# dotchen/LAV

Hardware: AMD Instinct MI355X
Metric: frames/s full agent fwd (32k-pt LiDAR + 3 cams) (higher is better)
Workload: dtype f32 (convolution contractions on the matrix cores with f32 accumulate at the error of an fp32 dot product, DESIGN 4.3: the layers on the split-operand kernel - BEV backbone, heads, crop stems, the brake net's mid-size layers - and ERFNet's persistent runs of pairs as two power-of-two-scaled fp16 pie

## Files before the change

include/lav_amd.h:

```cpp
#ifndef LAV_AMD_H
#define LAV_AMD_H

#include <stddef.h>
#include <stdint.h>

#ifdef __cplusplus
extern "C" {
#endif

#define LAV_ABI_VERSION 43

#define LAV_OK 0
#define LAV_EINVAL (-1)
#define LAV_EHIP (-2)
#define LAV_EWORKSPACE (-3)

int lav_abi_version(void);
const char *lav_last_error(void);
int lav_device_count(void);

int lav_profile_enable(int slots);
int lav_profile_reset(void);
int lav_profile_read(const char *kernel, double *total_ms, int *launches);

typedef struct lav_grid {
    float min_x, max_x, min_y, max_y;
    float ppm;
    int nx, ny;
} lav_grid;

typedef struct lav_pointnet {
    const float *w1, *b1, *w2, *b2;
    int num_input;
    int channels;
} lav_pointnet;

size_t lav_pillar_workspace_bytes(int batch, int max_points, const lav_grid *grid);
int lav_pillar_workspace_init(void *workspace, size_t workspace_bytes, void *stream);

int lav_pillar_scatter(const float *points, const int *h_num_points, int batch, int max_points, int D,
                       const lav_grid *grid, const lav_pointnet *net, float *canvas,
                       int *unique_coords, int *inverse, int *counts,
                       void *workspace, size_t workspace_bytes, void *stream);
// ... 75 lines not shown
                float *shift, void *stream);
int lav_conv_tile_info(const lav_conv *c, int *info);
size_t lav_conv_workspace_bytes(const lav_conv *c);
int lav_conv2d(const lav_conv *c, const float *x, const float *w_packed, const float *bias, const float *scale,
               const float *shift, const float *residual, float *y, void *workspace, size_t workspace_bytes,
               void *stream);
#define LAV_AMAX_PARTS 512
int lav_absmax_parts(const float *x, long n, float *parts, void *stream);
int lav_conv_amax_count(const lav_conv *c);
int lav_conv2d_amax(const lav_conv *c, const float *x, const float *w_packed, const float *bias, const float *scale,
                    const float *shift, const float *residual, float *y, void *workspace, size_t workspace_bytes,
                    const float *amax_in, int amax_in_count, float *amax_out, void *stream);

int lav_deconv_grouped(int batch, int cin, int h, int w, int groups, const int *cout_per_group, int kernel, int stride,
                       int pad, int out_pad, const float *x, const float *weight, const float *bias, int sigmoid_from,
                       float *y, void *stream);

int lav_crop_rotate(const float *feat, int feat_batch, int C, int H, int W, const float *locs, const float *oris, int n,
                    float pixels_per_meter, int crop, float offset_x, float offset_y, float *out, void *stream);
int lav_crop_rotate_indexed(const float *feat, int num_maps, const int *map_index, int C, int H, int W, const float *locs,
                            const float *oris, int n, float pixels_per_meter, int crop, float offset_x, float offset_y,
                            float *out, void *stream);
int lav_crop_rotate_backward(const float *grad_out, int num_maps, const int *map_index, int C, int H, int W, const float *locs,
                             const float *oris, int n, float pixels_per_meter, int crop, float offset_x, float offset_y,
                             float *grad_feat, void *stream);

int lav_merge_ticks(const float *tick, float *prev, int rows, int dim, float *cur, void *stream);
int lav_stack_sweeps(const float *fused, float *ring, const long *d_slot, const long *d_sweeps, const float *d_R,
                     const float *d_t, int num_sweeps, int rows, int dim, float *out, void *stream);
size_t lav_extract_peaks_workspace_bytes(int ncls, int h, int w);
int lav_extract_peaks(const float *heat, int ncls, int h, int w, int ks, int max_det, int apply_sigmoid,
                      const float *size, int size_c, const float *ori, int ori_c, float *out, void *workspace,
                      size_t workspace_bytes, void *stream);

int lav_attn_pool(const float *x, int batch, int C, int N, int heads, const float *u, const float *dots_bias,
                  const float *w_v, const float *b_v, float *out, void *stream);

size_t lav_attn_train_workspace_bytes(int batch, int C, int N, int heads);
int lav_attn_train_forward(const float *x, int batch, int C, int N, int heads, const float *q, const float *w_kv, const float *b_kv,
                           const float *pe, float scale, float *u, float *dots_bias, float *out, float *p, float *xbar, void *stream);
int lav_attn_train_backward(const float *x, int batch, int C, int N, int heads, const float *q, const float *w_kv, const float *b_kv,
                            const float *pe, float scale, const float *u, const float *p, const float *xbar, const float *dout, float *dx,
                            float *dq, float *dw_kv, float *db_kv, void *workspace, size_t workspace_bytes, void *stream);

int lav_nonfinite_count(int n, const float *const *tensors, const long *numel, int *counter2, void *stream);

int lav_maxpool3x3s2(const float *x, int batch, int channels, int h, int w, float *y, void *stream);
int lav_channel_affine(const float *x, int batch, int channels, long plane, const float *scale, const float *shift, float *y, void *stream);
int lav_copy_many(int n, const void *const *src, void *const *dst, const size_t *bytes, void *stream);
int lav_stage_many(int n, const void *const *src, float *const *dst, const int *dims, const long *strides, const int *src_is_u8,
                   void *stream);
int lav_stage_many_block(int n, const void *const *src, float *const *dst, const int *dims, const long *strides, const int *src_is_u8,
                         const void *block, int block_bytes, void *block_dst, void *stream);

int lav_linear_act(const float *x, int batch, int in_features, const float *weight, const float *bias, int out_features,
                   int act, float *out, void *stream);

int lav_det_decode(const float *rows, int ncls, int max_det, int cls, double min_score, double ego_x, double ego_y,
                   double near_px, double far_px, double min_box, double cx, double cy, double skip_px, double ppm,
                   float *actors, int *n_out, void *stream);
int lav_batch_limit(const int *d_rows);
int lav_det_decode_report(const float *rows, int ncls, int max_det, int cls, double min_score, double ego_x, double ego_y,
                          double near_px, double far_px, double min_box, double cx, double cy, double skip_px, double ppm,
                          float *actors, int *n_out, float *host_rows, int *host_n, unsigned *host_seq, void *stream);

size_t lav_pillar_decorate_workspace_bytes(int batch, int max_points, const lav_grid *grid);
// ... 182 lines not shown
```

lav_amd/_lib.py:

```python
from __future__ import annotations

import ctypes as C
import os

HERE = os.path.dirname(os.path.abspath(__file__))
LIB_PATH = os.environ.get("LAV_AMD_LIB") or os.path.join(HERE, "liblav_amd.so")

ABI_VERSION = 43
MAX_CAM = 4
MAX_CAM_F64 = 8


class Grid(C.Structure):
    _fields_ = [("min_x", C.c_float), ("max_x", C.c_float), ("min_y", C.c_float), ("max_y", C.c_float),
                ("ppm", C.c_float), ("nx", C.c_int), ("ny", C.c_int)]


class PointNet(C.Structure):
    _fields_ = [("w1", C.c_void_p), ("b1", C.c_void_p), ("w2", C.c_void_p), ("b2", C.c_void_p),
                ("num_input", C.c_int), ("channels", C.c_int)]


class Camera(C.Structure):
    _fields_ = [("K", C.c_float * 9), ("l2w", C.c_float * 16), ("w2c", C.c_float * 16)]


class CameraF64(C.Structure):
    _fields_ = [("l2w", C.c_double * 16), ("w2c", C.c_double * 16), ("K", C.c_double * 9)]


class Conv(C.Structure):
    _fields_ = [(n, C.c_int) for n in (
        "batch", "in_c_total", "in_c_offset", "cin", "h", "w", "cout", "kh", "kw", "stride", "pad_h", "pad_w",
        "dil_h", "dil_w", "transposed", "out_pad", "out_c_total", "out_c_offset", "relu_pre", "relu_post", "sigmoid", "target_cus")] + [("pad_value", C.c_float), ("precision", C.c_int)]


CONV_F32, CONV_BF16X6, CONV_F16X3 = 1, 2, 3


_P, _I, _Z, _F = C.c_void_p, C.c_int, C.c_size_t, C.c_float
SIGNATURES = {
# ... 77 lines not shown
    "lav_bn_train_forward_mask": (_I, [_P, _P, _P, _P, _I, _I, C.c_long, _P, _P, C.c_double, _I, _P, _P, _P, _P, _P, _Z, _P]),
    "lav_bn_train_backward_mask": (_I, [_P, _P, _P, _P, _I, _I, C.c_long, _P, _P, _P, _I, _P, _P, _P, _P, _P, _P, _Z, _P]),
    "lav_pair_train_supported": (_I, [_I, _I]),
    "lav_pair_train_workspace_bytes": (_Z, [_I, _I, _I]),
    "lav_pair_train_forward": (_I, [_P, _P, _P, _P, _P, _I, _I, _I, _I, _I, _P, _P, _P]),
    "lav_pair_train_backward": (_I, [_P, _P, _P, _P, _P, _I, _I, _I, _I, _I, _P, _P, _P, _P, _P, _P, _P, _Z, _P]),
    "lav_seg_xent_workspace_bytes": (_Z, []),
    "lav_seg_xent_forward": (_I, [_P, _P, _I, _I, C.c_long, _P, _P, _P, _Z, _P]),
    "lav_seg_xent_up_forward": (_I, [_P, _P, _I, _I, _I, _I, _I, _I, _P, _P, _P, _Z, _P]),
    "lav_attn_train_workspace_bytes": (_Z, [_I, _I, _I, _I]),
    "lav_attn_train_forward": (_I, [_P, _I, _I, _I, _I, _P, _P, _P, _P, C.c_float, _P, _P, _P, _P, _P, _P]),
    "lav_attn_train_backward": (_I, [_P, _I, _I, _I, _I, _P, _P, _P, _P, C.c_float, _P, _P, _P, _P, _P, _P, _P, _P, _P, _Z, _P]),
    "lav_bn_train_forward": (_I, [_P, _P, _P, _I, _I, C.c_long, _P, _P, C.c_double, _I, _I, _P, _P, _P, _P, _Z, _P]),
    "lav_bn_train_backward": (_I, [_P, _P, _P, _I, _I, C.c_long, _P, _P, _P, _I, _I, _P, _P, _P, _P, _P, _Z, _P]),
    "lav_bn_train_amax_count": (_I, [_I, _I, C.c_long]),
    "lav_bn_train_forward_amax": (_I, [_P, _P, _P, _I, _I, C.c_long, _P, _P, C.c_double, _I, _I, _P, _P, _P, _P, _P, _Z, _P]),
    "lav_bn_train_backward_amax": (_I, [_P, _P, _P, _I, _I, C.c_long, _P, _P, _P, _I, _I, _P, _P, _P, _P, _P, _P, _Z, _P]),
    "lav_attn_pool": (_I, [_P, _I, _I, _I, _I, _P, _P, _P, _P, _P, _P]),
    "lav_linear_act": (_I, [_P, _I, _I, _P, _P, _I, _I, _P, _P]),
    "lav_maxpool3x3s2": (_I, [_P, _I, _I, _I, _I, _P, _P]),
    "lav_channel_affine": (_I, [_P, _I, _I, C.c_long, _P, _P, _P, _P]),
    "lav_nonfinite_count": (_I, [_I, C.POINTER(_P), C.POINTER(C.c_long), _P, _P]),
    "lav_copy_many": (_I, [_I, C.POINTER(_P), C.POINTER(_P), C.POINTER(_Z), _P]),
    "lav_stage_many": (_I, [_I, C.POINTER(_P), C.POINTER(_P), C.POINTER(_I), C.POINTER(C.c_long), C.POINTER(_I), _P]),
    "lav_det_decode": (_I, [_P, _I, _I, _I] + [C.c_double] * 10 + [_P, _P, _P]),
    "lav_det_decode_report": (_I, [_P, _I, _I, _I] + [C.c_double] * 10 + [_P, _P, _P, _P, _P, _P]),
    "lav_stage_many_block": (_I, [_I, C.POINTER(_P), C.POINTER(_P), C.POINTER(_I), C.POINTER(C.c_long), C.POINTER(_I), _P, _I, _P, _P]),
    "lav_batch_limit": (_I, [_P]),
    "lav_pool_affine": (_I, [_P, _I, _I, _I, _I, _P, _P, _I, _P, _I, _I, _P]),
    "lav_merge_ticks": (_I, [_P, _P, _I, _I, _P, _P]),
    "lav_stack_sweeps": (_I, [_P, _P, _P, _P, _P, _P, _I, _I, _I, _P, _P]),
    "lav_extract_peaks_workspace_bytes": (_Z, [_I, _I, _I]),
    "lav_extract_peaks": (_I, [_P, _I, _I, _I, _I, _I, _I, _P, _I, _P, _I, _P, _P, _Z, _P]),
    "lav_augment_u8": (_I, [_P, _P, _I, _I, _I, _P, C.c_ulonglong, _P]),
    "lav_bev_stack_u8": (_I, [_P, _P, _P, _P, _I, _I, _I, _I, _P]),
    "lav_bev_stack_tile_paths": (_I, [C.POINTER(C.c_double), C.POINTER(_I), _I, _I, C.POINTER(_I)]),
    "lav_debug_view": (_I, [_P, _I, _I, _P, _I, _I, _P, _I, _I, _P, _I, _P, _I, _P, _I, _P, _P, _P, C.c_double, C.c_double, _I, C.c_double, C.c_double, _I,
                            _I, _I, _P, _P, _P]),
    "lav_log_view": (_I, [_P, _I, _P, _I, _P, _P, _I, _I, _P, _P, _I, _P, _I, _I, _P, _P]),
    "lav_eval_acc_words": (_Z, [_I]),
    "lav_eval_frame": (_I, [_P, _P, _P, _I, _I, _F, _P, _I, _P, _P, _I, _I, _I, _P, _P, _I, _P, _P, _P, _I] + [C.c_double] * 6 + [_I, _P, _P]),
    "lav_eval_seg": (_I, [_P, _P, _I, _I, _I, _I, _I, _P, _P]),
    "lav_eval_scores": (_I, [_P, _P, _I, C.c_double, _I, _P, _P]),
    "lav_eval_plans_words": (_Z, [_I]),
    "lav_eval_plans": (_I, [_P, _P, _P, _P, _P, _P, _I, _I, _I, _P, _P, _P, _I, _P, _P]),
    "lav_eval_distill_words": (_Z, [_I]),
    "lav_eval_distill": (_I, [_P] * 8 + [_I, _I, _I] + [_P] * 5 + [_I, _P, _P]),
    "lav_eval_drive_words": (_Z, [_I]),
    "lav_eval_drive": (_I, [_P, _P, _P, _I, _I, _I, _I, _P, _P, _I, _P, _P, _I, _I] + [C.c_double] * 6 + [_I, _P, _P]),
    "lav_jpeg_scan_capacity": (C.c_longlong, [_I, _I, _I]),
    "lav_jpeg_workspace_bytes": (_Z, [_I, _I, _I, _I]),
    "lav_jpeg_encode": (_I, [_P, _I, _I, _I, _I, _P, _I, _P, C.c_longlong, _P, _P, _Z, _P]),
}

_lib = None


def load() -> C.CDLL:
    global _lib
    if _lib is not None:
        return _lib
    if not os.path.exists(LIB_PATH):
        raise RuntimeError(
            f"{LIB_PATH} not found: build it with `python -m lav_amd.build` (hipcc, gfx950). "
            "lav_amd has no CPU or pure-torch fallback.")
    lib = C.CDLL(LIB_PATH)
# ... 24 lines not shown
```

lav_amd/build.py:

```python
from __future__ import annotations

import os
import subprocess
import sys
import time

HERE = os.path.dirname(os.path.abspath(__file__))
REPO = os.path.dirname(HERE)
CSRC = os.path.join(HERE, "csrc")
LIB = os.path.join(HERE, "liblav_amd.so")
SOURCES = ["misc.hip", "pillar.hip", "paint.hip", "paint_frames.hip", "gru.hip", "gru_seq.hip", "conv.hip", "conv_f16.hip", "conv_pair.hip", "conv_run.hip", "conv_tile.hip", "deconv.hip", "crop.hip", "frame.hip", "attn.hip", "bn_train.hip", "conv_wgrad.hip", "upconv.hip", "conv_pair_train.hip", "augment.hip", "bev_stack.hip", "debug_view.hip", "log_view.hip", "eval_metrics.hip", "eval_camera.hip", "eval_plans.hip", "eval_drive.hip", "eval_distill.hip", "jpeg.hip"]
EXTRA_FLAGS = {"pillar.hip": ["-ffp-contract=off"], "paint.hip": ["-ffp-contract=off"], "paint_frames.hip": ["-ffp-contract=off"], "crop.hip": ["-ffp-contract=off"],
               "frame.hip": ["-ffp-contract=off"], "augment.hip": ["-ffp-contract=off"], "bev_stack.hip": ["-ffp-contract=off"],
               "debug_view.hip": ["-ffp-contract=off", "-fhip-fp32-correctly-rounded-divide-sqrt"],
               "log_view.hip": ["-ffp-contract=off"],
               "eval_metrics.hip": ["-ffp-contract=off"],
               "eval_plans.hip": ["-ffp-contract=off"],
               "eval_drive.hip": ["-ffp-contract=off"],
               "eval_distill.hip": ["-ffp-contract=off"]}
FLAGS = ["--offload-arch=gfx950", "-O3", "-std=c++17", "-fPIC", "-Wall", "-Wno-unused-function", "-fno-slp-vectorize",
         "-I", os.path.join(REPO, "include"), "-I", CSRC]


def _hipcc() -> str:
    for c in (os.environ.get("HIPCC"), "/opt/rocm/bin/hipcc", "hipcc"):
        if c and (os.path.isabs(c) and os.path.exists(c) or not os.path.isabs(c)):
            return c
    raise RuntimeError("hipcc not found")


def needs_build() -> bool:
    if not os.path.exists(LIB):
        return True
    t = os.path.getmtime(LIB)
    deps = [os.path.join(CSRC, f) for f in os.listdir(CSRC)] + [os.path.join(REPO, "include", "lav_amd.h")]
    return any(os.path.getmtime(d) > t for d in deps)


def build(force: bool = False, verbose: bool = True) -> str:
    if not force and not needs_build():
        return LIB
    objs = []
    procs = []
    os.makedirs(os.path.join(HERE, "build"), exist_ok=True)
# ... 24 lines not shown
```

lav_amd/frame.py:

```python
from __future__ import annotations

import math
import os
import time
from collections import deque

import numpy as np
import torch

from . import ops
from .model_inference import InferModel

GAP = 5
_COPY_STREAM = os.environ.get("LAV_COPY_STREAM", "0") == "1"
_DET_REPORT = os.environ.get("LAV_DET_REPORT", "1") != "0"
_POSE_BLOCK = os.environ.get("LAV_POSE_BLOCK", "1") != "0"
_BRAKE_AFTER = os.environ.get("LAV_BRAKE_AFTER", "in")
_BRAKE_SPLIT = os.environ.get("LAV_BRAKE_SPLIT", "wide")
if _BRAKE_SPLIT in ("0", "off", "none"):
    _BRAKE_SPLIT = ""
_DIAG_SKIP = set(filter(None, os.environ.get("LAV_DIAG_SKIP", "").split(",")))


def ego_box_mask(lidar: torch.Tensor) -> torch.Tensor:
    x, y, z = lidar[:, 0], lidar[:, 1], lidar[:, 2]
    return (x > -2.4) & (x < 0) & (y > -0.8) & (y < 0.8) & (z > -1.5) & (z < -1)


def move_lidar_points(xyz: torch.Tensor, dloc, ori0: float, ori1: float) -> torch.Tensor:
    dloc = np.asarray(dloc, np.float64) @ np.array([[math.cos(ori0), -math.sin(ori0)], [math.sin(ori0), math.cos(ori0)]])
    ori = ori1 - ori0
    c, s_ = float(np.float32(math.cos(ori))), float(np.float32(math.sin(ori)))
    x, y = xyz[:, 0], xyz[:, 1]
    return torch.stack([(x * c + y * -s_) + float(np.float32(dloc[0])), (x * s_ + y * c) + float(np.float32(dloc[1])),
                        xyz[:, 2]], dim=1)


def _at_frame_precision(fn):
    import functools

    @functools.wraps(fn)
    def wrapped(self, *a, **k):
        with ops.precision(self.precision):
            return fn(self, *a, **k)
    return wrapped


class FramePipeline:
    def __init__(self, lidar_model, uniplanner, seg_model, bra_model, camera_x=1.5, camera_z=2.4, num_frame_stack=2,
                 device=torch.device("cuda"), compact_ego_box: bool = False):
        self.device = device
        self.precision = ops.frame_precision()
        self.infer_model = InferModel(lidar_model, uniplanner, camera_x, camera_z, device=device, precision=self.precision)
        self.seg_model, self.bra_model = seg_model, bra_model
        self.num_frame_stack = num_frame_stack
        self.num_frame_keep = (num_frame_stack + 1) * GAP
        self.compact_ego_box = compact_ego_box
        self.reset()

    def reset(self):
        self.lidars, self.locs, self.oris = deque(), deque(), deque()
        self.prev_lidar = None

    def _sem_probs(self, all_rgbs):
        probs = getattr(self.seg_model, "probs", None)
        return probs(all_rgbs) if probs is not None else torch.softmax(self.seg_model(all_rgbs), dim=1)

    def preprocess(self, lidar):
        m = ego_box_mask(lidar)
        if self.compact_ego_box:
            return lidar[~m]
        out = lidar.clone()
        out[:, 0] = torch.where(m, torch.full_like(out[:, 0], float("nan")), out[:, 0])
        return out

    def get_stacked_lidar(self):
        loc0, ori0 = self.locs[-1], self.oris[-1]
        parts = []
        for i, t in enumerate(range(len(self.lidars) - 1, -1, -GAP)):
            lidar = self.lidars[t]
            xyz = move_lidar_points(lidar[:, :3], self.locs[t] - loc0, ori0, self.oris[t])
            onehot = torch.zeros((len(xyz), self.num_frame_stack + 1), dtype=xyz.dtype, device=xyz.device)
            onehot[:, i] = 1
            parts.append(torch.cat([xyz, lidar[:, 3:], onehot], dim=-1))
        return torch.cat(parts)

# ... 80 lines not shown

    def _grow(self, new_p: int):
        torch.cuda.synchronize()
        f = dict(dtype=torch.float32, device=self.device)
        old_p = self.P
        b_tick = torch.full((new_p, 4), float("nan"), **f)
        b_prev = torch.full((new_p, 4), float("nan"), **f); b_prev[:old_p] = self.b_prev
        ring = torch.full((self.num_frame_keep, 2 * new_p, 8), float("nan"), **f); ring[:, :2 * old_p] = self.ring
        self.b_tick, self.b_prev, self.ring, self.P = b_tick, b_prev, ring, new_p
        self.graphs.clear(); self.outs.clear()
        torch.cuda.synchronize()

    def reset(self):
        super().reset()
        if hasattr(self, "ring"):
            self.ring.fill_(float("nan")); self.b_prev.fill_(float("nan"))
            self.frame_no = 0
            self.poses = deque()

    def _g_lidar(self):
        im, lm = self.infer_model, self.infer_model.lidar_model
        cur = ops.merge_ticks(self.b_tick, self.b_prev)
        pred_sem = self._sem_probs(self.b_all_rgbs)
        fused = im.forward_paint(cur, pred_sem)
        lidar_points = ops.stack_sweeps(fused, self.ring, self.b_slot, self.b_sweeps, self.b_R, self.b_t)
        canvas = lm.point_pillar_net([lidar_points], [lidar_points.shape[0]])
        if self.b_features is None:
            self.b_features = torch.empty((1, lm.backbone.out_channels, canvas.shape[2] // 2, canvas.shape[3] // 2),
                                          dtype=torch.float32, device=canvas.device)
        lm.backbone(canvas, out=self.b_features)
        return dict(lidar_points=lidar_points)

    def _g_heads(self):
        heat, size, ori, pred_bev = self.infer_model.lidar_model.heads(self.b_features)
        det_raw = ops.extract_peaks(heat[0], size[0], ori[0], apply_sigmoid=True)
        if self.device_others:
            im, up = self.infer_model, self.infer_model.uniplanner
            ox, oy = up.offsets()
            H, W = im._bev_hw
            ops.det_decode(det_raw, self.d_actors, self.d_n, cls=1, min_score=0.2, ego_xy=(160, 280), near_px=2.0,
                           far_px=30 * im.pixels_per_meter, min_box=0.1 * im.pixels_per_meter,
                           centre_xy=(float(W / 2 + ox * W / 2), float(H / 2 + oy * H / 2)), skip_px=4.0, ppm=up.pixels_per_meter,
                           report=(self.h_det, self.h_n, self.h_seq) if _DET_REPORT else None)
            if self.forced_others is not None:
                self.d_actors.copy_(self.forced_others[0]); self.d_n.copy_(self.forced_others[1])
        return dict(det_raw=det_raw, pred_bev=pred_bev)

    def set_forced_others(self, locs=None, oris=None):
        if not self.device_others:
            raise RuntimeError("set_forced_others needs the device-resident others branch")
        if locs is None:
            self.forced_others = None
        else:
            n = len(locs)
            host = torch.zeros((45,), dtype=torch.float32)
            host[:2 * n] = torch.as_tensor(locs, dtype=torch.float32).reshape(-1)
            host[30:30 + n] = torch.as_tensor(oris, dtype=torch.float32).reshape(-1)
            self.forced_others = (host.to(self.device), torch.tensor([n], dtype=torch.int32, device=self.device), n)
        torch.cuda.synchronize()
        self.graphs.pop("heads", None); self.outs.pop("heads", None)

    def _g_brake(self):
        pred_bra = self.bra_model(self.b_rgbs, self.b_tel)
        ops.nonfinite_count([pred_bra], self.d_health)
        return dict(pred_bra=pred_bra)

    def _g_brake_a(self):
        first = self.b_rgbs if _BRAKE_SPLIT == "wide" else self.b_tel
# ... 303 lines not shown
```

lav_amd/lidar.py:

```python
from __future__ import annotations

import torch
from torch import nn
import torch.nn.functional as F

from . import _lib
from . import ops
from .engine import Engine, _bn_tuple
from .ops import Amax, ConvLayer, ConvRun, ConvTileRun, GroupedDeconv, PointwiseUpconv
from .point_pillar import PointPillarNet

_NORM = dict(eps=1e-3, momentum=0.01)


def _stage(cin, cout, n):
    mods = []
    for j in range(n):
        mods += [nn.Conv2d(cin if j == 0 else cout, cout, 3, 2 if j == 0 else 1, 1, bias=False),
                 nn.ReLU(inplace=True), nn.BatchNorm2d(cout, **_NORM)]
    return nn.Sequential(*mods)


def _up(cin, cout, k, s, p=0, op=0):
    return nn.Sequential(nn.ConvTranspose2d(cin, cout, k, s, p, op, bias=False), nn.ReLU(inplace=True),
# ... 148 lines not shown
        self.seg_head = Head(6 * nf, 3, output_activation=torch.sigmoid)

    def _head_engine(self, names, device):
        prec = ops.infer_precision()
        if prec == 0 and getattr(self, "heads_precision", 0):
            prec = self.heads_precision
        def build():
            hs = [getattr(self, n) for n in names]
            for h in hs:
                if not (h._sigmoid or isinstance(h.output_activation, nn.Identity)):
                    raise RuntimeError("Head.output_activation must be identity or sigmoid for the fused epilogue")
            sig = [h._sigmoid for h in hs]
            if any(sig[:-1]):
                raise RuntimeError("fused head deconvolution expects the sigmoid head last")
            w = lambda: torch.cat([h.net[0].weight.detach() for h in hs], dim=0)
            bn = lambda: tuple(torch.cat([getattr(h.net[2], n).detach() for h in hs]) for n in ("running_mean", "running_var", "weight", "bias"))
            cts = [h.net[3] for h in hs]
            outs = [ct.weight.shape[1] for ct in cts]
            return dict(outs=outs,
                        conv=ConvLayer(w, padding=1, bn=bn, bn_eps=hs[0].net[2].eps, relu_pre=True, device=device,
                                       precision=prec),
                        deconv=GroupedDeconv(cts, sigmoid_from=sum(outs[:-1]) if sig[-1] else -1, device=device))
        return self._engine_for(device, (names, prec), build)

    ALL_HEADS = ("center_head", "box_head", "ori_head", "seg_head")

    def heads(self, features, names=ALL_HEADS):
        if self.training:
            return self._heads_train(features, names)
        e = self._head_engine(tuple(names), features.device)
        fused = e["deconv"](e["conv"](features, amax_in=ops.amax_of(features)))
        return tuple(torch.split(fused, e["outs"], dim=1))

    def _heads_train(self, features, names):
        hs = [getattr(self, n) for n in names]
        if len(hs) == 1 or not features.is_cuda:
            return tuple(h(features) for h in hs)
        from .train.hipnn import bn_act_many, conv2d
        mid = conv2d(features, torch.cat([h.net[0].weight for h in hs], dim=0), 1, 1)
        mid = bn_act_many([h.net[2] for h in hs], mid, relu_pre=True)
        outs, off = [], 0
        for h in hs:
            c = h.net[0].out_channels
            outs.append(h.output_activation(h.net[3](mid[:, off:off + c])))
            off += c
        return tuple(outs)

    def forward(self, lidars, num_points):
        features = self.backbone(self.point_pillar_net(lidars, num_points))
        return (features, *self.heads(features))
```

lav_amd/model_inference.py:

```python
from __future__ import annotations

import numpy as np
import torch
import torch.nn as nn
from torch.nn import functional as F

from . import ops
from .planner_common import crop_feature, transform_points

CAMERA_YAWS = [-60, 0, 60]


def carla_matrix(x, y, z, yaw_deg=0.0):
    f = np.float32
    a = f(yaw_deg) * (f(np.pi) / f(180.0))
    c, s = np.cos(a, dtype=f), np.sin(a, dtype=f)
    return np.array([[c, -s, 0, x], [s, c, 0, y], [0, 0, 1, z], [0, 0, 0, 1]], f)


def carla_inverse_matrix(x, y, z, yaw_deg=0.0):
    f = np.float32
    a = f(yaw_deg) * (f(np.pi) / f(180.0))
    c, s = np.cos(a, dtype=f), np.sin(a, dtype=f)
    ax, ay, az = -f(x), -f(y), -f(z)
# ... 7 lines not shown

    def __init__(self, cam_yaw, lidar_xyz=(0, 0, 2.5), cam_xyz=(1.4, 0, 2.5), rgb_h=320, rgb_w=320, fov=60):
        super().__init__()
        focal = rgb_w / (2.0 * np.tan(fov * np.pi / 360.0))
        K = torch.eye(3)
        K[0, 0] = K[1, 1] = focal
        K[0, 2] = rgb_w / 2.0
        K[1, 2] = rgb_h / 2.0
        self.K = nn.Parameter(K, requires_grad=False)
        self.lidar_to_world = nn.Parameter(torch.from_numpy(carla_matrix(*lidar_xyz)), requires_grad=False)
        self.world_to_cam = nn.Parameter(torch.from_numpy(carla_inverse_matrix(*cam_xyz, yaw_deg=cam_yaw)), requires_grad=False)
        self.rgb_h, self.rgb_w = rgb_h, rgb_w

    def matrices(self):
        return (self.K.detach().cpu().numpy(), self.lidar_to_world.detach().cpu().numpy(),
                self.world_to_cam.detach().cpu().numpy())

    def forward(self, lidar):
        sem = torch.zeros((1, 5, self.rgb_h, self.rgb_w), dtype=torch.float32, device=lidar.device)
        _, uvz = ops.paint(lidar, sem, ops.make_cameras([self.matrices()]), want_uvz=True)
        return uvz[0].long()


def extract_peak(heatmap, max_pool_ks: int = 7, min_score: float = 0.1, max_det: int = 15, break_tie: bool = False):
    if break_tie:
        heatmap = heatmap + 1e-7 * torch.randn(*heatmap.size(), device=heatmap.device)
    h, w = heatmap.shape
    z = heatmap.new_zeros((1, h, w))
    rows = ops.extract_peaks(heatmap[None].contiguous(), z, z, ks=max_pool_ks, max_det=min(max_det, h * w)).cpu()
    return [(float(s), int(x), int(y)) for s, x, y in rows[0, :, :3].tolist() if s > min_score]


class InferModel(nn.Module):
    def __init__(self, lidar_model, uniplanner, camera_x, camera_z, device=torch.device("cuda"), precision=None):
        super().__init__()
        self.precision = ops.frame_precision() if precision is None else int(precision)
        self.lidar_model = lidar_model
        self.uniplanner = uniplanner
        self.coord_converters = [CoordConverter(yaw, lidar_xyz=[0, 0, camera_z], cam_xyz=[camera_x, 0, camera_z],
                                                rgb_h=288, rgb_w=256, fov=64) for yaw in CAMERA_YAWS]
        self._cams = ops.make_cameras([cc.matrices() for cc in self.coord_converters])
        self.pixels_per_meter = uniplanner.pixels_per_meter
        self.offset_x, self.offset_y = uniplanner.offset_x, uniplanner.offset_y
        self.crop_size = uniplanner.crop_size
        self.num_cmds, self.num_plan = uniplanner.num_cmds, uniplanner.num_plan
        self.plan, self.cast, self.cast_cmd_pred = uniplanner.plan, uniplanner.cast, uniplanner.cast_cmd_pred
        ny, nx = lidar_model.point_pillar_net.ny, lidar_model.point_pillar_net.nx
        self._bev_hw = (int(ny), int(nx))

    @torch.no_grad()
    def forward_paint(self, cur_lidar, pred_sem):
        return ops.paint(cur_lidar, pred_sem, self._cams)

    @torch.no_grad()
    def forward(self, lidar_points, nxps, cmd_value):
        lm = self.lidar_model
        with ops.precision(self.precision):
            canvas = lm.point_pillar_net([lidar_points], [len(lidar_points)])
            features = lm.backbone(canvas)
            heat, size, ori, pred_bev = lm.heads(features)
            det = self.det_decode(ops.extract_peaks(heat[0], size[0], ori[0], apply_sigmoid=True).cpu().tolist())
            ego_embd, ego_plan, ego_cast, other_cast, other_cmds = self.uniplanner.infer_all(features[0], det[1], cmd_value, nxps, amax=ops.amax_of(features))
        return ego_embd, ego_plan, ego_cast, other_cast, other_cmds, pred_bev, det

    def det_inference(self, heatmaps, sizemaps, orimaps, min_score=0.2):
        return self.det_decode(ops.extract_peaks(heatmaps, sizemaps, orimaps).cpu().tolist(), min_score)

    def det_decode(self, det_rows, min_score=0.2):
        dets = []
        for i, rows in enumerate(det_rows):
            det = []
            for s, x, y, w, h, cos, sin in rows:
                if not s > min_score:
                    continue
                x, y = int(x), int(y)
                if i == 1 and max(w, h) < 0.1 * self.pixels_per_meter:
                    continue
                dist = np.linalg.norm([x - 160, y - 280])
                if dist <= 2 or dist >= 30 * self.pixels_per_meter:
                    continue
                det.append((x, y, w, h, cos, sin))
            dets.append(det)
        return dets

    def det_decode_fast(self, rows: np.ndarray, min_score=0.2):
        ppm = self.pixels_per_meter
        rows64 = rows.astype(np.float64)
        s, x, y = rows64[..., 0], rows[..., 1].astype(np.int64), rows[..., 2].astype(np.int64)
        w, h = rows64[..., 3], rows64[..., 4]
        dist = np.sqrt(((x - 160) ** 2 + (y - 280) ** 2).astype(np.float64))
        keep = (s > min_score) & (dist > 2) & (dist < 30 * ppm)
        if rows.shape[0] > 1:
            keep[1] &= ~(np.maximum(w[1], h[1]) < 0.1 * ppm)
        dets = [[(int(x[i, j]), int(y[i, j]), float(w[i, j]), float(h[i, j]), float(rows[i, j, 5]), float(rows[i, j, 6]))
# ... 24 lines not shown
```

lav_amd/ops.py:

```python
from __future__ import annotations

import ctypes as C
import os as _os
import threading as _threading
from typing import Optional, Sequence

import numpy as np
import torch

from . import _lib
from ._lib import Camera, Conv, Grid, PointNet, check

_workspaces: dict = {}


def _stream() -> int:
    return torch.cuda.current_stream().cuda_stream


def _ptr(t: Optional[torch.Tensor]) -> Optional[int]:
    return None if t is None else t.data_ptr()


def _f32c(t: torch.Tensor, name: str) -> torch.Tensor:
# ... 757 lines not shown
    words = (C.c_int * 16)()
    check(lib.lav_gru_plan_diag(_ptr(ws), ws.numel(), B, H, num_cmds, cmd, words, st.cuda_stream), "lav_gru_plan_diag")
    return dict(zip(names, list(words)))


_precision_stack = _threading.local()


def infer_precision() -> int:
    st = getattr(_precision_stack, "v", None)
    if st:
        return st[-1]
    return {"f16x3": _lib.CONV_F16X3, "bf16x6": _lib.CONV_BF16X6, "f32": _lib.CONV_F32, "fp32": _lib.CONV_F32}.get(
        _os.environ.get("LAV_INFER_PRECISION", ""), 0)


class precision:

    def __init__(self, p: int):
        self.p = int(p)

    def __enter__(self):
        st = getattr(_precision_stack, "v", None)
        if st is None:
            st = _precision_stack.v = []
        st.append(self.p)
        return self

    def __exit__(self, *exc):
        _precision_stack.v.pop()
        return False


def frame_precision() -> int:
    if _os.environ.get("LAV_CONV_PRECISION", "") in ("f32", "fp32"):
        return 0
    want = _os.environ.get("LAV_INFER_PRECISION", _os.environ.get("LAV_HEADS_PRECISION", "f16x3"))
    return _lib.CONV_F16X3 if want == "f16x3" else 0


class Amax:
    CAPACITY = 20480

    def __init__(self, device, capacity: Optional[int] = None, zeroed: bool = True):
        self.CAPACITY = int(capacity) if capacity else Amax.CAPACITY
        self.buf = (torch.zeros if zeroed else torch.empty)(self.CAPACITY, dtype=torch.float32, device=device)
        self.count = 0
        self.generation = 0

    def reset(self):
        self.count = 0
        self.generation += 1
        return self

    def take(self, n: int) -> torch.Tensor:
        if self.count + n > self.CAPACITY:
            raise RuntimeError(f"Amax: {self.count} + {n} parts exceed the buffer ({self.CAPACITY})")
        v = self.buf[self.count:self.count + n]
        self.count += n
        return v


def tag_amax(t, am):
    if am is None:
        return t
    t._lav_amax = am
# ... 725 lines not shown
    if fb not in (1, n):
        raise RuntimeError("features batch must be 1 (shared map) or N")
    check(lib.lav_crop_rotate(_ptr(features), fb, Cc, H, W, _ptr(locs), _ptr(oris), n, float(pixels_per_meter), int(crop),
                              float(offset_x), float(offset_y), _ptr(out), _stream()), "lav_crop_rotate")
    return out


def merge_ticks(tick: torch.Tensor, prev: torch.Tensor, out: torch.Tensor | None = None) -> torch.Tensor:
    lib = _lib.load()
    tick, prev = _f32c(tick, "tick"), _f32c(prev, "prev")
    if tick.shape != prev.shape or tick.dim() != 2 or tick.shape[1] != 4:
        raise RuntimeError(f"merge_ticks: tick {tuple(tick.shape)} / prev {tuple(prev.shape)} must both be (P, 4)")
    P = tick.shape[0]
    if out is None:
        out = torch.empty((2 * P, 4), dtype=torch.float32, device=tick.device)
    check(lib.lav_merge_ticks(_ptr(tick), _ptr(prev), P, 4, _ptr(out), _stream()), "lav_merge_ticks")
    return out


def stack_sweeps(fused: torch.Tensor, ring: torch.Tensor, slot: torch.Tensor, sweeps: torch.Tensor, R: torch.Tensor,
                 t: torch.Tensor, out: torch.Tensor | None = None) -> torch.Tensor:
    lib = _lib.load()
    fused, ring, R, t = _f32c(fused, "fused"), _f32c(ring, "ring"), _f32c(R, "R"), _f32c(t.reshape(-1, 3), "t")
    S, rows, dim = sweeps.numel(), fused.shape[0], fused.shape[1]
    if ring.shape[1:] != fused.shape or slot.dtype != torch.long or sweeps.dtype != torch.long or R.shape != (S, 3, 3):
        raise RuntimeError("stack_sweeps: inconsistent arguments")
    if out is None:
        out = torch.empty((S * rows, dim + S), dtype=torch.float32, device=fused.device)
    check(lib.lav_stack_sweeps(_ptr(fused), _ptr(ring), _ptr(slot), _ptr(sweeps), _ptr(R), _ptr(t), S, rows, dim, _ptr(out),
                               _stream()), "lav_stack_sweeps")
    return out


def extract_peaks(heat: torch.Tensor, size: torch.Tensor, ori: torch.Tensor, ks: int = 7, max_det: int = 15,
                  apply_sigmoid: bool = False) -> torch.Tensor:
    lib = _lib.load()
    heat, size, ori = _f32c(heat, "heat"), _f32c(size, "size"), _f32c(ori, "ori")
    ncls, H, W = heat.shape
    if size.shape[1:] != (H, W) or ori.shape[1:] != (H, W):
        raise RuntimeError("extract_peaks: size / ori maps must match the heat map")
    out = torch.empty((ncls, max_det, 3 + size.shape[0] + ori.shape[0]), dtype=torch.float32, device=heat.device)
    nbytes = lib.lav_extract_peaks_workspace_bytes(ncls, H, W)
    ws = _workspace("peaks", nbytes, heat.device)
    check(lib.lav_extract_peaks(_ptr(heat), ncls, H, W, ks, max_det, int(apply_sigmoid), _ptr(size), size.shape[0], _ptr(ori),
                                ori.shape[0], _ptr(out), _ptr(ws), ws.numel(), _stream()), "lav_extract_peaks")
    return out
```

Measured before the change: 536.2.

## Evaluate box and orientation heads only at detected peak locations

```diff
diff --git a/include/lav_amd.h b/include/lav_amd.h
--- a/include/lav_amd.h
+++ b/include/lav_amd.h
@@ -8,7 +8,7 @@
 extern "C" {
 #endif
 
-#define LAV_ABI_VERSION 43
+#define LAV_ABI_VERSION 44
 
 #define LAV_OK 0
 #define LAV_EINVAL (-1)
@@ -150,6 +150,11 @@
 int lav_extract_peaks(const float *heat, int ncls, int h, int w, int ks, int max_det, int apply_sigmoid,
                       const float *size, int size_c, const float *ori, int ori_c, float *out, void *workspace,
                       size_t workspace_bytes, void *stream);
+
+size_t lav_heads_at_peaks_packed_floats(int cin, int hidden);
+int lav_heads_at_peaks(const float *feat, int cin, int h, int w, const float *rows, int ncls, int max_det, int nheads,
+                       const float *const *w1_packed, const float *const *scale, const float *const *shift, const float *const *wt,
+                       const float *const *bias, const int *hidden, const int *outs, float *out, void *stream);
 
 int lav_attn_pool(const float *x, int batch, int C, int N, int heads, const float *u, const float *dots_bias,
                   const float *w_v, const float *b_v, float *out, void *stream);
diff --git a/lav_amd/_lib.py b/lav_amd/_lib.py
--- a/lav_amd/_lib.py
+++ b/lav_amd/_lib.py
@@ -6,7 +6,7 @@
 HERE = os.path.dirname(os.path.abspath(__file__))
 LIB_PATH = os.environ.get("LAV_AMD_LIB") or os.path.join(HERE, "liblav_amd.so")
 
-ABI_VERSION = 43
+ABI_VERSION = 44
 MAX_CAM = 4
 MAX_CAM_F64 = 8
 
@@ -150,6 +150,8 @@
     "lav_stack_sweeps": (_I, [_P, _P, _P, _P, _P, _P, _I, _I, _I, _P, _P]),
     "lav_extract_peaks_workspace_bytes": (_Z, [_I, _I, _I]),
     "lav_extract_peaks": (_I, [_P, _I, _I, _I, _I, _I, _I, _P, _I, _P, _I, _P, _P, _Z, _P]),
+    "lav_heads_at_peaks_packed_floats": (_Z, [_I, _I]),
+    "lav_heads_at_peaks": (_I, [_P, _I, _I, _I, _P, _I, _I, _I, _P, _P, _P, _P, _P, _P, _P, _P, _P]),
     "lav_augment_u8": (_I, [_P, _P, _I, _I, _I, _P, C.c_ulonglong, _P]),
     "lav_bev_stack_u8": (_I, [_P, _P, _P, _P, _I, _I, _I, _I, _P]),
     "lav_bev_stack_tile_paths": (_I, [C.POINTER(C.c_double), C.POINTER(_I), _I, _I, C.POINTER(_I)]),
diff --git a/lav_amd/build.py b/lav_amd/build.py
--- a/lav_amd/build.py
+++ b/lav_amd/build.py
@@ -9,7 +9,7 @@
 REPO = os.path.dirname(HERE)
 CSRC = os.path.join(HERE, "csrc")
 LIB = os.path.join(HERE, "liblav_amd.so")
-SOURCES = ["misc.hip", "pillar.hip", "paint.hip", "paint_frames.hip", "gru.hip", "gru_seq.hip", "conv.hip", "conv_f16.hip", "conv_pair.hip", "conv_run.hip", "conv_tile.hip", "deconv.hip", "crop.hip", "frame.hip", "attn.hip", "bn_train.hip", "conv_wgrad.hip", "upconv.hip", "conv_pair_train.hip", "augment.hip", "bev_stack.hip", "debug_view.hip", "log_view.hip", "eval_metrics.hip", "eval_camera.hip", "eval_plans.hip", "eval_drive.hip", "eval_distill.hip", "jpeg.hip"]
+SOURCES = ["misc.hip", "pillar.hip", "paint.hip", "paint_frames.hip", "gru.hip", "gru_seq.hip", "conv.hip", "conv_f16.hip", "conv_pair.hip", "conv_run.hip", "conv_tile.hip", "deconv.hip", "crop.hip", "frame.hip", "heads_peaks.hip", "attn.hip", "bn_train.hip", "conv_wgrad.hip", "upconv.hip", "conv_pair_train.hip", "augment.hip", "bev_stack.hip", "debug_view.hip", "log_view.hip", "eval_metrics.hip", "eval_camera.hip", "eval_plans.hip", "eval_drive.hip", "eval_distill.hip", "jpeg.hip"]
 EXTRA_FLAGS = {"pillar.hip": ["-ffp-contract=off"], "paint.hip": ["-ffp-contract=off"], "paint_frames.hip": ["-ffp-contract=off"], "crop.hip": ["-ffp-contract=off"],
                "frame.hip": ["-ffp-contract=off"], "augment.hip": ["-ffp-contract=off"], "bev_stack.hip": ["-ffp-contract=off"],
                "debug_view.hip": ["-ffp-contract=off", "-fhip-fp32-correctly-rounded-divide-sqrt"],
diff --git a/lav_amd/csrc/heads_peaks.hip b/lav_amd/csrc/heads_peaks.hip
--- /dev/null
+++ b/lav_amd/csrc/heads_peaks.hip
@@ -0,0 +1,172 @@
+#include "common.hpp"
+
+namespace {
+using namespace lav;
+
+constexpr int HP_THREADS = 1024, HP_HID = 64, HP_CC = 384, HP_MAX_HEADS = 4, HP_MAX_OUTS = 4;
+constexpr int HP_SLICE = 256 + 8;
+
+__device__ __forceinline__ void add_carry(float &s, float &c, float x) {
+    const float t = s + x, bb = t - s;
+    c += (s - (t - bb)) + (x - bb);
+    s = t;
+}
+
+__device__ __forceinline__ float lane_xor32(float v) {
+    const unsigned u = __float_as_uint(v);
+    const auto a = __builtin_amdgcn_permlane32_swap(u, u, false, false);
+    return __uint_as_float(a[0] ^ a[1] ^ u);
+}
+__device__ __forceinline__ float lane_xor16(float v) {
+    const unsigned u = __float_as_uint(v);
+    const auto a = __builtin_amdgcn_permlane16_swap(u, u, false, false);
+    return __uint_as_float(a[0] ^ a[1] ^ u);
+}
+
+struct HeadsPeaksArgs {
+    const float *feat, *rows;
+    float *out;
+    int cin, H, W, nrows, ncol, nheads;
+    const float *w1[HP_MAX_HEADS];
+    const float *scale[HP_MAX_HEADS], *shift[HP_MAX_HEADS];
+    const float *wt[HP_MAX_HEADS];
+    const float *bias[HP_MAX_HEADS];
+    int hidden[HP_MAX_HEADS], outs[HP_MAX_HEADS], col[HP_MAX_HEADS];
+};
+
+__global__ __launch_bounds__(HP_THREADS) void k_heads_at_peaks(HeadsPeaksArgs a) {
+    __shared__ float s_patch[HP_CC * 16];
+    __shared__ float s_part[32 * HP_SLICE];
+    __shared__ float s_hid[HP_HID * 4];
+    __shared__ float s_tail[HP_MAX_OUTS * HP_HID];
+    const int tid = threadIdx.x, row = blockIdx.x, g = blockIdx.y;
+    const float *r = a.rows + (long)row * 3;
+    const float score = r[0], fx = r[1], fy = r[2];
+    const bool live = score > -1e4f && fx >= 0.f && fx < (float)(2 * a.W) && fy >= 0.f && fy < (float)(2 * a.H);
+    const int x = min(max(live ? (int)fx : 0, 0), 2 * a.W - 1), y = min(max(live ? (int)fy : 0, 0), 2 * a.H - 1);
+    const int hx0 = x >> 1, hy0 = y >> 1;
+    const int K = 9 * a.cin, kpad = (K + 127) / 128 * 128;
+    const float *w1 = a.w1[g];
+    const int lane = tid & 63, wv = tid >> 6, k8 = lane >> 3, c8 = lane & 7;
+
+    float acc[8][4];
+#pragma unroll
+    for (int c = 0; c < 8; ++c)
+#pragma unroll
+        for (int p = 0; p < 4; ++p) acc[c][p] = 0.f;
+
+    for (int c0 = 0; c0 < a.cin; c0 += HP_CC) {
+        const int cn = min(HP_CC, a.cin - c0);
+        for (int e = tid; e < cn * 16; e += HP_THREADS) {
+            const int ci = c0 + (e >> 4), yy = hy0 - 1 + ((e >> 2) & 3), xx = hx0 - 1 + (e & 3);
+            const bool in = yy >= 0 && yy < a.H && xx >= 0 && xx < a.W;
+            const long at = in ? ((long)ci * a.H + yy) * a.W + xx : 0;
+            const float v = a.feat[at];
+            s_patch[e] = in ? v : 0.f;
+        }
+        __syncthreads();
+        const int kb = 9 * c0, kn = min(9 * cn, kpad - kb), kr = (kn + 127) / 128 * 128;
+        const float4 *wp = reinterpret_cast<const float4 *>(w1 + (long)(kb + 8 * wv + k8) * HP_HID + 8 * c8);
+#pragma unroll 3
+        for (int kk = 8 * wv + k8; kk < kr; kk += 128, wp += 128 * HP_HID / 4) {
+            const float4 w0 = wp[0], w4 = wp[1];
+            const int kc = min(kk, kn - 1), ci = kc / 9, t = kc - ci * 9, ky = t / 3, kx = t - ky * 3;
+            const float *f = s_patch + ci * 16 + ky * 4 + kx;
+            const float f0 = kk < kn ? f[0] : 0.f, f1 = kk < kn ? f[1] : 0.f, f2 = kk < kn ? f[4] : 0.f, f3 = kk < kn ? f[5] : 0.f;
+            const float wc[8] = {w0.x, w0.y, w0.z, w0.w, w4.x, w4.y, w4.z, w4.w};
+#pragma unroll
+            for (int c = 0; c < 8; ++c) {
+                acc[c][0] = fmaf(wc[c], f0, acc[c][0]);
+                acc[c][1] = fmaf(wc[c], f1, acc[c][1]);
+                acc[c][2] = fmaf(wc[c], f2, acc[c][2]);
+                acc[c][3] = fmaf(wc[c], f3, acc[c][3]);
+            }
+        }
+        __syncthreads();
+    }
+#pragma unroll
+    for (int c = 0; c < 8; ++c)
+#pragma unroll
+        for (int p = 0; p < 4; ++p) {
+            float v = acc[c][p];
+            v = v + lane_xor32(v);
+            v = v + lane_xor16(v);
+            if (k8 < 2) s_part[(wv * 2 + k8) * HP_SLICE + (c * 4 + p) * 8 + c8] = v;
+        }
+    __syncthreads();
+    const int hid = a.hidden[g], outs = a.outs[g];
+    if (tid < 256) {
+        float v = s_part[tid], carry = 0.f;
+        for (int s = 1; s < 32; ++s) add_carry(v, carry, s_part[s * HP_SLICE + tid]);
+        v += carry;
+        const int j = tid >> 3, ch = 8 * (tid & 7) + (j >> 2), p = j & 3;
+        const bool have = ch < hid;
+        const float sc = a.scale[g][have ? ch : 0], sh = a.shift[g][have ? ch : 0];
+        s_hid[ch * 4 + p] = have ? fmaf(fmaxf(v, 0.f), sc, sh) : 0.f;
+    }
+    __syncthreads();
+    if (tid < outs * HP_HID) {
+        const int o = tid >> 6, ch = tid & 63;
+        float t = 0.f;
+        if (ch < hid) {
+            const float *w = a.wt[g] + ((long)ch * outs + o) * 9;
+#pragma unroll
+            for (int p = 0; p < 4; ++p) {
+                const int py = p >> 1, px = p & 1;
+                const bool use = (py == 0 || ((y & 1) && hy0 + 1 < a.H)) && (px == 0 || ((x & 1) && hx0 + 1 < a.W));
+                const int ky = (y & 1) ? (py ? 0 : 2) : 1, kx = (x & 1) ? (px ? 0 : 2) : 1;
+                const float wv_ = w[ky * 3 + kx];
+                t = use ? fmaf(s_hid[ch * 4 + p], wv_, t) : t;
+            }
+        }
+        s_tail[tid] = t;
+    }
+    __syncthreads();
+    float *orow = a.out + (long)row * a.ncol;
+    if (tid < outs) {
+        float v = s_tail[tid * HP_HID], carry = 0.f;
+        for (int ch = 1; ch < HP_HID; ++ch) add_carry(v, carry, s_tail[tid * HP_HID + ch]);
+        if (a.bias[g]) add_carry(v, carry, a.bias[g][tid]);
+        orow[a.col[g] + tid] = live ? v + carry : 0.f;
+    }
+    if (g == 0 && tid >= 64 && tid < 67) orow[tid - 64] = r[tid - 64];
+}
+}
+
+extern "C" size_t lav_heads_at_peaks_packed_floats(int cin, int hidden) {
+    if (cin < 1 || hidden < 1 || hidden > HP_HID) return 0;
+    return (size_t)((9l * cin + 127) / 128 * 128) * HP_HID;
+}
+
+extern "C" int lav_heads_at_peaks(const float *feat, int cin, int h, int w, const float *rows, int ncls, int max_det, int nheads,
+                                  const float *const *w1_packed, const float *const *scale, const float *const *shift,
+                                  const float *const *wt, const float *const *bias, const int *hidden, const int *outs, float *out,
+                                  void *stream) {
+    LAV_REQUIRE(feat && rows && out && w1_packed && scale && shift && wt && bias && hidden && outs, "lav_heads_at_peaks: null argument");
+    LAV_REQUIRE(cin >= 1 && h >= 1 && w >= 1 && (long)cin * h * w < (1l << 31) && h < (1 << 29) && w < (1 << 29), "lav_heads_at_peaks: bad map size");
+    LAV_REQUIRE(ncls >= 1 && max_det >= 1 && (long)ncls * max_det <= 65535, "lav_heads_at_peaks: bad row count");
+    LAV_REQUIRE(nheads >= 1 && nheads <= HP_MAX_HEADS, "lav_heads_at_peaks: 1 .. %d heads", HP_MAX_HEADS);
+    HeadsPeaksArgs a;
+    a.feat = feat; a.rows = rows; a.out = out;
+    a.cin = cin; a.H = h; a.W = w; a.nrows = ncls * max_det; a.nheads = nheads;
+    int col = 3;
+    for (int g = 0; g < HP_MAX_HEADS; ++g) {
+        const bool on = g < nheads;
+        if (on) {
+            LAV_REQUIRE(hidden[g] >= 1 && hidden[g] <= HP_HID && outs[g] >= 1 && outs[g] <= HP_MAX_OUTS,
+                        "lav_heads_at_peaks: head %d: hidden width in 1 .. %d and 1 .. %d outputs expected", g, HP_HID, HP_MAX_OUTS);
+            LAV_REQUIRE(w1_packed[g] && scale[g] && shift[g] && wt[g], "lav_heads_at_peaks: head %d: null weights", g);
+        }
+        a.w1[g] = on ? w1_packed[g] : nullptr; a.scale[g] = on ? scale[g] : nullptr; a.shift[g] = on ? shift[g] : nullptr;
+        a.wt[g] = on ? wt[g] : nullptr; a.bias[g] = on ? bias[g] : nullptr;
+        a.hidden[g] = on ? hidden[g] : 0; a.outs[g] = on ? outs[g] : 0; a.col[g] = col;
+        col += a.outs[g];
+    }
+    a.ncol = col;
+    hipStream_t st = static_cast<hipStream_t>(stream);
+    const int tok = timer_begin("heads_at_peaks", st);
+    hipLaunchKernelGGL(k_heads_at_peaks, dim3(a.nrows, nheads), dim3(HP_THREADS), 0, st, a);
+    timer_end(tok, st);
+    LAV_LAUNCH_CHECK();
+    return LAV_OK;
+}
diff --git a/lav_amd/frame.py b/lav_amd/frame.py
--- a/lav_amd/frame.py
+++ b/lav_amd/frame.py
@@ -19,7 +19,8 @@
 _BRAKE_SPLIT = os.environ.get("LAV_BRAKE_SPLIT", "wide")
 if _BRAKE_SPLIT in ("0", "off", "none"):
     _BRAKE_SPLIT = ""
-_DIAG_SKIP = set(filter(None, os.environ.get("LAV_DIAG_SKIP", "").split(",")))
+_HEADS_AT_PEAKS = ops.frame_heads_at_peaks()
+_DIAG_SKIP =set(filter(None, os.environ.get("LAV_DIAG_SKIP", "").split(",")))
 
 
 def ego_box_mask(lidar: torch.Tensor) -> torch.Tensor:
@@ -51,7 +52,8 @@
                  device=torch.device("cuda"), compact_ego_box: bool = False):
         self.device = device
         self.precision = ops.frame_precision()
-        self.infer_model = InferModel(lidar_model, uniplanner, camera_x, camera_z, device=device, precision=self.precision)
+        self.infer_model = InferModel(lidar_model, uniplanner, camera_x, camera_z, device=device, precision=self.precision,
+                                      heads_at_peaks=_HEADS_AT_PEAKS)
         self.seg_model, self.bra_model = seg_model, bra_model
         self.num_frame_stack = num_frame_stack
         self.num_frame_keep = (num_frame_stack + 1) * GAP
@@ -198,8 +200,7 @@
         return dict(lidar_points=lidar_points)
 
     def _g_heads(self):
-        heat, size, ori, pred_bev = self.infer_model.lidar_model.heads(self.b_features)
-        det_raw = ops.extract_peaks(heat[0], size[0], ori[0], apply_sigmoid=True)
+        det_raw, pred_bev = self.infer_model.lidar_model.detect(self.b_features, at_peaks=self.infer_model.heads_at_peaks)
         if self.device_others:
             im, up = self.infer_model, self.infer_model.uniplanner
             ox, oy = up.offsets()
diff --git a/lav_amd/lidar.py b/lav_amd/lidar.py
--- a/lav_amd/lidar.py
+++ b/lav_amd/lidar.py
@@ -204,6 +204,22 @@
         fused = e["deconv"](e["conv"](features, amax_in=ops.amax_of(features)))
         return tuple(torch.split(fused, e["outs"], dim=1))
 
+    def detect(self, features, at_peaks=True):
+        if features.shape[0] != 1:
+            raise RuntimeError("LiDARModel.detect: one frame (batch 1) expected")
+        if not at_peaks:
+            heat, size, ori, pred_bev = self.heads(features)
+            return ops.extract_peaks(heat[0], size[0], ori[0], apply_sigmoid=True), pred_bev
+        heat, pred_bev = self.heads(features, ("center_head", "seg_head"))
+        rows = ops.extract_peaks(heat[0], apply_sigmoid=True)
+        names = ("box_head", "ori_head")
+        def build():
+            hs = [getattr(self, n) for n in names]
+            if not all(isinstance(h.output_activation, nn.Identity) for h in hs):
+                raise RuntimeError("LiDARModel.detect: the box / orientation heads must have no output activation")
+            return ops.HeadsAtPeaks([(h.net[0], h.net[2], h.net[3]) for h in hs], device=features.device)
+        return self._engine_for(features.device, ("at_peaks", names), build)(features[0], rows), pred_bev
+
     def _heads_train(self, features, names):
         hs = [getattr(self, n) for n in names]
         if len(hs) == 1 or not features.is_cuda:
diff --git a/lav_amd/model_inference.py b/lav_amd/model_inference.py
--- a/lav_amd/model_inference.py
+++ b/lav_amd/model_inference.py
@@ -63,9 +63,10 @@
 
 
 class InferModel(nn.Module):
-    def __init__(self, lidar_model, uniplanner, camera_x, camera_z, device=torch.device("cuda"), precision=None):
+    def __init__(self, lidar_model, uniplanner, camera_x, camera_z, device=torch.device("cuda"), precision=None, heads_at_peaks=None):
         super().__init__()
         self.precision = ops.frame_precision() if precision is None else int(precision)
+        self.heads_at_peaks = ops.frame_heads_at_peaks() if heads_at_peaks is None else bool(heads_at_peaks)
         self.lidar_model = lidar_model
         self.uniplanner = uniplanner
         self.coord_converters = [CoordConverter(yaw, lidar_xyz=[0, 0, camera_z], cam_xyz=[camera_x, 0, camera_z],
@@ -89,8 +90,8 @@
         with ops.precision(self.precision):
             canvas = lm.point_pillar_net([lidar_points], [len(lidar_points)])
             features = lm.backbone(canvas)
-            heat, size, ori, pred_bev = lm.heads(features)
-            det = self.det_decode(ops.extract_peaks(heat[0], size[0], ori[0], apply_sigmoid=True).cpu().tolist())
+            det_rows, pred_bev = lm.detect(features, at_peaks=self.heads_at_peaks)
+            det = self.det_decode(det_rows.cpu().tolist())
             ego_embd, ego_plan, ego_cast, other_cast, other_cmds = self.uniplanner.infer_all(features[0], det[1], cmd_value, nxps, amax=ops.amax_of(features))
         return ego_embd, ego_plan, ego_cast, other_cast, other_cmds, pred_bev, det
 
diff --git a/lav_amd/ops.py b/lav_amd/ops.py
--- a/lav_amd/ops.py
+++ b/lav_amd/ops.py
@@ -813,6 +813,10 @@
         return False
 
 
+def frame_heads_at_peaks() -> bool:
+    return _os.environ.get("LAV_HEADS_AT_PEAKS", "1") != "0"
+
+
 def frame_precision() -> int:
     if _os.environ.get("LAV_CONV_PRECISION", "") in ("f32", "fp32"):
         return 0
@@ -1604,16 +1608,83 @@
     return out
 
 
-def extract_peaks(heat: torch.Tensor, size: torch.Tensor, ori: torch.Tensor, ks: int = 7, max_det: int = 15,
-                  apply_sigmoid: bool = False) -> torch.Tensor:
-    lib = _lib.load()
-    heat, size, ori = _f32c(heat, "heat"), _f32c(size, "size"), _f32c(ori, "ori")
+def extract_peaks(heat: torch.Tensor, size: Optional[torch.Tensor] = None, ori: Optional[torch.Tensor] = None, ks: int = 7,
+                  max_det: int = 15, apply_sigmoid: bool = False) -> torch.Tensor:
+    lib = _lib.load()
+    heat = _f32c(heat, "heat")
+    size, ori = (None if size is None else _f32c(size, "size")), (None if ori is None else _f32c(ori, "ori"))
     ncls, H, W = heat.shape
-    if size.shape[1:] != (H, W) or ori.shape[1:] != (H, W):
+    if any(m is not None and m.shape[1:] != (H, W) for m in (size, ori)):
         raise RuntimeError("extract_peaks: size / ori maps must match the heat map")
-    out = torch.empty((ncls, max_det, 3 + size.shape[0] + ori.shape[0]), dtype=torch.float32, device=heat.device)
+    cs, co = (0 if size is None else size.shape[0]), (0 if ori is None else ori.shape[0])
+    out = torch.empty((ncls, max_det, 3 + cs + co), dtype=torch.float32, device=heat.device)
     nbytes = lib.lav_extract_peaks_workspace_bytes(ncls, H, W)
     ws = _workspace("peaks", nbytes, heat.device)
-    check(lib.lav_extract_peaks(_ptr(heat), ncls, H, W, ks, max_det, int(apply_sigmoid), _ptr(size), size.shape[0], _ptr(ori),
-                                ori.shape[0], _ptr(out), _ptr(ws), ws.numel(), _stream()), "lav_extract_peaks")
+    check(lib.lav_extract_peaks(_ptr(heat), ncls, H, W, ks, max_det, int(apply_sigmoid), _ptr(size), cs, _ptr(ori), co, _ptr(out),
+                                _ptr(ws), ws.numel(), _stream()), "lav_extract_peaks")
     return out
+
+
+class HeadsAtPeaks:
+
+    def __init__(self, heads, device=None):
+        lib = _lib.load()
+        self._heads = [tuple(h) for h in heads]
+        conv0, _, ct0 = self._heads[0]
+        if not 1 <= len(self._heads) <= 4:
+            raise RuntimeError("HeadsAtPeaks: 1 .. 4 heads")
+        for conv, bn, ct in self._heads:
+            if (conv.kernel_size, conv.stride, conv.padding, conv.dilation, conv.groups, conv.in_channels) != ((3, 3), (1, 1), (1, 1), (1, 1), 1, conv0.in_channels) \
+                    or conv.bias is not None or conv.padding_mode != "zeros":
+                raise RuntimeError("HeadsAtPeaks: first layer must be Conv2d(cin, hidden, 3, 1, 1, bias=False)")
+            if (ct.kernel_size, ct.stride, ct.padding, ct.output_padding, ct.dilation, ct.groups, ct.in_channels) != \
+                    ((3, 3), (2, 2), (1, 1), (1, 1), (1, 1), 1, conv.out_channels) or bn.num_features != conv.out_channels:
+                raise RuntimeError("HeadsAtPeaks: tail must be ConvTranspose2d(hidden, outs, 3, 2, 1, 1) behind a BatchNorm2d(hidden)")
+        self._dev = device if device is not None else conv0.weight.device
+        self.cin = conv0.in_channels
+        self.hidden = [conv.out_channels for conv, _, _ in self._heads]
+        self.outs = [ct.out_channels for _, _, ct in self._heads]
+        n = [lib.lav_heads_at_peaks_packed_floats(self.cin, h) for h in self.hidden]
+        if not all(n) or max(self.outs) > 4:
+            raise RuntimeError("HeadsAtPeaks: hidden width <= 64 and at most 4 outputs per head")
+        f = dict(dtype=torch.float32, device=self._dev)
+        self.w1 = [torch.zeros((k // 64, 64), **f) for k in n]
+        self.scale = [torch.empty((h,), **f) for h in self.hidden]
+        self.shift = [torch.empty((h,), **f) for h in self.hidden]
+        self.wt = [torch.empty((h, o, 3, 3), **f) for h, o in zip(self.hidden, self.outs)]
+        self.bias = [None if ct.bias is None else torch.empty((o,), **f) for (_, _, ct), o in zip(self._heads, self.outs)]
+        self.refresh()
+        G = len(self._heads)
+        arr = lambda ts: (C.c_void_p * G)(*[_ptr(t) for t in ts])
+        self._args = (arr(self.w1), arr(self.scale), arr(self.shift), arr(self.wt), arr(self.bias), (C.c_int * G)(*self.hidden),
+                      (C.c_int * G)(*self.outs))
+
+    def refresh(self):
+        for g, (conv, bn, ct) in enumerate(self._heads):
+            hid = self.hidden[g]
+            w = conv.weight.detach().to(self._dev, torch.float32)
+            self.w1[g][:9 * self.cin, :hid].copy_(w.permute(1, 2, 3, 0).reshape(9 * self.cin, hid))
+            scale, shift = bn_fold(*[t.detach().cpu() for t in (bn.running_mean, bn.running_var, bn.weight, bn.bias)], bn.eps)
+            self.scale[g].copy_(scale.to(torch.float32))
+            self.shift[g].copy_(shift.to(torch.float32))
+            self.wt[g].copy_(ct.weight.detach())
+            if self.bias[g] is not None:
+                self.bias[g].copy_(ct.bias.detach())
+
+    def __call__(self, feat: torch.Tensor, rows: torch.Tensor, out: Optional[torch.Tensor] = None) -> torch.Tensor:
+        feat, rows = _f32c(feat, "feat"), _f32c(rows, "rows")
+        if feat.dim() != 3 or feat.shape[0] != self.cin or rows.dim() != 3 or rows.shape[2] != 3:
+            raise RuntimeError(f"heads_at_peaks: feature map (cin = {self.cin}, H, W) and rows (ncls, max_det, 3) expected")
+        ncls, max_det = rows.shape[:2]
+        shape = (ncls, max_det, 3 + sum(self.outs))
+        if out is None:
+            out = torch.empty(shape, dtype=torch.float32, device=feat.device)
+        elif tuple(out.shape) != shape or not out.is_contiguous() or out.dtype != torch.float32:
+            raise RuntimeError(f"heads_at_peaks: output buffer must be contiguous float32 {shape}")
+        check(_lib.load().lav_heads_at_peaks(_ptr(feat), self.cin, feat.shape[1], feat.shape[2], _ptr(rows), ncls, max_det,
+                                            len(self._heads), *self._args, _ptr(out), _stream()), "lav_heads_at_peaks")
+        return out
+
+
+def heads_at_peaks(layer: HeadsAtPeaks, feat: torch.Tensor, rows: torch.Tensor) -> torch.Tensor:
+    return layer(feat, rows)
```

New measurement: 552.0, median of 6. 2.9% higher.
